# AaltoML/SLAM-module

Measured on AMD Instinct MI355X. Metric: frames/sec ORB extract+match (720p), higher is better.
Workload: dtype u8

## Files before the change

### slam-module_amd/csrc/describe_lanes.h

```cpp
#pragma once
#include <cstdint>

namespace describe_lanes {

constexpr int kWinRows = 45, kWinDwords = 12, kWinPieces = 9;
constexpr int kPatchRows = 32, kPatchDwords = 8, kHalfPatch = 15;
constexpr int kOriRow0 = 7, kOriDword0 = 2;

constexpr uint32_t win_pack(int lane) {
    uint32_t p = 0;
    for (int b = 0; b < 3; ++b) {
        const int i = lane + 64 * b;
        p |= (uint32_t)((i / kWinDwords) | ((4 * (i % kWinDwords)) << 4)) << (10 * b);
    }
    return p;
}
constexpr int win_row(uint32_t pack, int t) { return (int)((pack >> (10 * (t % 3))) & 15u) + 16 * (t / 3); }
constexpr int win_byte(uint32_t pack, int t) { return (int)((pack >> (10 * (t % 3) + 4)) & 63u); }
constexpr bool win_active(int lane, int t) { return t < kWinPieces - 1 || lane < kWinRows * kWinDwords - 64 * (kWinPieces - 1); }
constexpr int win_src_row(uint32_t pack, int lane, int t) { return win_active(lane, t) ? win_row(pack, t) : 16 * (t / 3); }
constexpr int win_src_byte(uint32_t pack, int lane, int t) { return win_active(lane, t) ? win_byte(pack, t) : 0; }
constexpr int win_slot(int lane, int t) { return lane + 64 * t; }
constexpr int kSlabDwords = kWinRows * kWinDwords + kPatchRows * kPatchDwords + 4;

constexpr int ori_base(int lane) { return ((lane >> 3) + kOriRow0) * kWinDwords + (lane & 7) + kOriDword0; }
constexpr int ori_src(int lane, int t) { return ori_base(lane) + 8 * kWinDwords * t; }
constexpr int ori_dst(int lane, int t) { return lane + 64 * t; }
constexpr bool ori_active(int lane, int t) { return t < 3 || lane < (kPatchRows - 1) * kPatchDwords - 64 * 3; }

inline uint32_t disc_mask(int lane, int t, const int *u_max) {
    const int i = ori_dst(lane, t), r = i >> 3, c4 = i & 7;
    if (r >= kPatchRows - 1) return 0u;
    uint32_t m = 0;
    for (int b = 0; b < 4; ++b) {
        const int u = 4 * c4 + b - kHalfPatch, v = r - kHalfPatch;
        if (u <= kHalfPatch && (u < 0 ? -u : u) <= u_max[v < 0 ? -v : v]) m |= 0xFFu << (8 * b);
    }
    return m;
}

constexpr uint32_t moment_col_weights(int lane) { return 0x03020100u + 0x04040404u * (uint32_t)(lane & 7); }
constexpr int moment_row_bias(int lane) { return (lane >> 3) - kHalfPatch + 24; }

#if defined(__HIP_DEVICE_COMPILE__)
__device__ __forceinline__ uint32_t sad_u8(uint32_t a, uint32_t acc) { return __builtin_amdgcn_sad_u8(a, 0u, acc); }
__device__ __forceinline__ uint32_t dot4_u8(uint32_t a, uint32_t w, uint32_t acc) { return __builtin_amdgcn_udot4(a, w, acc, false); }
#define DESCRIBE_LANES_FN __device__ __forceinline__
#else
inline uint32_t sad_u8(uint32_t a, uint32_t acc) { return acc + (a & 255u) + ((a >> 8) & 255u) + ((a >> 16) & 255u) + (a >> 24); }
inline uint32_t dot4_u8(uint32_t a, uint32_t w, uint32_t acc) {
    for (int b = 0; b < 4; ++b) acc += ((a >> (8 * b)) & 255u) * ((w >> (8 * b)) & 255u);
    return acc;
}
#define DESCRIBE_LANES_FN inline
#endif

DESCRIBE_LANES_FN void lane_moments(const uint32_t (&d)[4], uint32_t col_weights, int row_bias, int &m10, int &m01) {
    const uint32_t p0 = sad_u8(d[0], 0u), p1 = sad_u8(d[1], p0), p2 = sad_u8(d[2], p1), T = sad_u8(d[3], p2);
    const uint32_t D = dot4_u8(d[3], col_weights, dot4_u8(d[2], col_weights, dot4_u8(d[1], col_weights, dot4_u8(d[0], col_weights, 0u))));
    m10 = (int)D - kHalfPatch * (int)T;
    m01 = row_bias * (int)T - 8 * (int)(p0 + p1 + p2);
}
#undef DESCRIBE_LANES_FN

constexpr int kTapZeroSlot = 16;
constexpr int tap_slot(int lane, int t) {
    return ((unsigned)(lane - 16 * t) < 32u && (t < 2 || (lane & 15) <= 6)) ? lane - 16 * t : kTapZeroSlot;
}
inline void tap_table(uint32_t *out ) {
    const int w7[7] = {18, 34, 48, 56, 48, 34, 18};
    for (int i = 0; i < 64 * 4; ++i) out[i] = 0u;
    for (int tab = 0; tab < 2; ++tab)
        for (int dt = 0; dt < 2; ++dt)
            for (int n = 0; n < 16; ++n)
                for (int j = 0; j < 16; ++j) {
                    const int tap = 16 * dt + j - n - (tab == 0 ? 1 : 0);
                    const uint32_t v = (tap >= 0 && tap <= 6) ? (uint32_t)w7[tap] : 0u;
                    out[((tab * 2 + dt) * 16 + n) * 4 + j / 4] |= v << (8 * (j % 4));
                }
}

}
```

### slam-module_amd/csrc/hamming_fp4.h

```cpp
#pragma once
#include <stdint.h>

#if defined(__HIPCC__)
#define HM4_HD __host__ __device__ __forceinline__
#else
#define HM4_HD inline
#endif

constexpr uint32_t kHm4ScaleA = 0x80808080u;
constexpr uint32_t kHm4ScaleB = 0x83838383u;
constexpr int kHm4Steps = 4;

struct Hm4Slot { int step, half, dword, nibble; };
HM4_HD Hm4Slot hm4_slot(int bit) {
    const int wi = bit >> 5, b = bit & 31;
    return Hm4Slot{wi >> 1, wi & 1, b & 3, b >> 2};
}
HM4_HD uint32_t hm4_target_dword(uint32_t w, int j) { return (w >> j) & 0x11111111u; }
HM4_HD uint32_t hm4_query_dword(uint32_t w, int j) { return ((j < 3 ? w << (3 - j) : w) & 0x88888888u) | 0x22222222u; }
```

### slam-module_amd/csrc/match.hip

```cpp
#include "ms_internal.h"
#include "hamming_fp4.h"
#include <algorithm>
#include <cmath>
#include <cstring>
#include <vector>

namespace {

constexpr uint32_t kNone = 0xFFFFFFFFu;

__device__ __forceinline__ uint32_t hamming8(const uint32_t q[8], const uint4 a, const uint4 b) {
    uint32_t d = __popc(q[0] ^ a.x);
    d += __popc(q[1] ^ a.y); d += __popc(q[2] ^ a.z); d += __popc(q[3] ^ a.w);
    d += __popc(q[4] ^ b.x); d += __popc(q[5] ^ b.y); d += __popc(q[6] ^ b.z); d += __popc(q[7] ^ b.w);
    return d;
}

struct HamArgs {
    const uint32_t *q, *t;
    int32_t q_stride, t_stride;
    const int32_t *q_count, *t_count;
    const int32_t *pair_q, *pair_t;
    int32_t nq, nt;
    const int32_t *qb, *tb;
// ... 22 lines not shown
    int32_t my_bucket = 0;
    if (qi < nq) {
        const uint4 a = Q[2 * qi], b = Q[2 * qi + 1];
        qr[0] = a.x; qr[1] = a.y; qr[2] = a.z; qr[3] = a.w; qr[4] = b.x; qr[5] = b.y; qr[6] = b.z; qr[7] = b.w;
        if (MASKED && A.qb) my_bucket = A.qb[(uint64_t)qs * A.q_stride + qi];
    }
    uint32_t best = kNone, second = kNone;
    for (int base = 0; base < nt; base += 256) {
        __syncthreads();
        const int j = base + tid;
        if (j < nt) {
            s_t[tid][0] = T[2 * j]; s_t[tid][1] = T[2 * j + 1];
            if (MASKED) {
                s_b[tid] = A.tb ? A.tb[(uint64_t)ts * A.t_stride + j] : 0;
                s_v[tid] = A.tv ? A.tv[(uint64_t)ts * A.t_stride + j] : 1;
            }
        }
        __syncthreads();
        const int cnt = min(256, nt - base);
        for (int k = 0; k < cnt; ++k) {
            const uint32_t d = hamming8(qr, s_t[k][0], s_t[k][1]);
            uint32_t key = (d << 20) | (uint32_t)(base + k);
            if (MASKED) {
                const bool ok = s_v[k] != 0 && (!(A.qb && A.tb) || s_b[k] == my_bucket);
                key = ok ? key : kNone;
            }
            const uint32_t lo = min(best, key), hi = max(best, key);
            second = min(second, hi);
            best = lo;
        }
    }
    if (qi < A.q_stride) {
        const bool live = qi < nq;
        A.best_idx[o] = (!live || best == kNone) ? -1 : (int32_t)(best & 0xFFFFFu);
        A.best_dist[o] = (!live || best == kNone) ? (uint16_t)MS_HAMMING_MAX : (uint16_t)(best >> 20);
        A.second_dist[o] = (!live || second == kNone) ? (uint16_t)MS_HAMMING_MAX : (uint16_t)(second >> 20);
    }
}

typedef int v4i_t __attribute__((ext_vector_type(4)));
typedef int v8i_t __attribute__((ext_vector_type(8)));
typedef float v16f_t __attribute__((ext_vector_type(16)));
typedef unsigned short us2_t __attribute__((ext_vector_type(2)));
constexpr int kHmStage = 128;
static_assert(kHmStage == 128 || kHmStage == 256, "the expansion below gives every thread kHmStage / 128 sixteen-byte loads");

__device__ __forceinline__ void best2_push(uint32_t &best, uint32_t &second, uint32_t key) {
    const uint32_t lo = min(best, key), hi = max(best, key);
    second = min(second, hi);
    best = lo;
}
__device__ __forceinline__ v8i_t hm_operand(v4i_t v) { return v8i_t{v[0], v[1], v[2], v[3], 0, 0, 0, 0}; }

__global__ __launch_bounds__(256) void k_hamming_mfma(HamArgs A) {
    __shared__ __attribute__((aligned(16))) uint32_t s_a[kHmStage * 32];
    const int p = blockIdx.y, tid = threadIdx.x, lane = tid & 63, wave = __builtin_amdgcn_readfirstlane(tid >> 6);
    const int col = lane & 31, h = lane >> 5;
    const int qs = A.pair_q ? A.pair_q[p] : p, ts = A.pair_t ? A.pair_t[p] : p;
    const int nq = A.q_count ? min(A.q_count[qs], A.nq) : A.nq;
    const int nt = A.t_count ? min(A.t_count[ts], A.nt) : A.nt;
    if (blockIdx.x * 256 >= nq) {
        const int qi = blockIdx.x * 256 + tid;
        const uint64_t o = (uint64_t)p * A.q_stride + qi;
        if (qi < A.q_stride) { A.best_idx[o] = -1; A.best_dist[o] = MS_HAMMING_MAX; A.second_dist[o] = MS_HAMMING_MAX; }
        return;
    }
    const uint4 *Q = reinterpret_cast<const uint4 *>(A.q + (uint64_t)qs * A.q_stride * 8);
    const uint4 *T = reinterpret_cast<const uint4 *>(A.t + (uint64_t)ts * A.t_stride * 8);
    v4i_t bq[2][kHm4Steps];
    int popq[2];
    const uint32_t hmask = 0u - (uint32_t)h;
#pragma unroll
    for (int n = 0; n < 2; ++n) {
        const int qi = blockIdx.x * 256 + wave * 64 + n * 32 + col;
        uint4 lo = {0, 0, 0, 0}, hi = {0, 0, 0, 0};
        if (qi < nq) { lo = Q[2 * qi]; hi = Q[2 * qi + 1]; }
        const uint32_t w[8] = {lo.x, lo.y, lo.z, lo.w, hi.x, hi.y, hi.z, hi.w};
#pragma unroll
        for (int s = 0; s < kHm4Steps; ++s) {
            const uint32_t wq = (w[2 * s + 1] & hmask) | (w[2 * s] & ~hmask);
#pragma unroll
            for (int j = 0; j < 4; ++j) bq[n][s][j] = (int)hm4_query_dword(wq, j);
        }
        popq[n] = 0;
#pragma unroll
        for (int s = 0; s < 8; ++s) popq[n] += __popc(w[s]);
    }
    uint32_t best[2] = {kNone, kNone}, second[2] = {kNone, kNone};
    v16f_t tag;
#pragma unroll
    for (int r = 0; r < 16; ++r) tag[r] = 8388608.0f + 4096.0f + (float)r;
    for (int base = 0; base < nt; base += kHmStage) {
        __syncthreads();
#pragma unroll
        for (int it = 0; it < kHmStage / 128; ++it) {
            const int e = tid + 256 * it, tau = e % kHmStage, half = e / kHmStage, j = base + tau;
            uint4 v = {0, 0, 0, 0};
            if (j < nt) v = T[2 * j + half];
            const uint32_t w4[4] = {v.x, v.y, v.z, v.w};
#pragma unroll
            for (int k = 0; k < 4; ++k)
                *reinterpret_cast<v4i_t *>(&s_a[((tau >> 5) * kHm4Steps + 2 * half + (k >> 1)) * 256 + ((k & 1) * 32 + (tau & 31)) * 4]) =
                    v4i_t{(int)hm4_target_dword(w4[k], 0), (int)hm4_target_dword(w4[k], 1), (int)hm4_target_dword(w4[k], 2), (int)hm4_target_dword(w4[k], 3)};
        }
        __syncthreads();
        const int mtiles = min(kHmStage / 32, (nt - base + 31) >> 5);
        for (int m = 0; m < mtiles; ++m) {
            v16f_t acc[2];
            v4i_t a[kHm4Steps];
#pragma unroll
            for (int s = 0; s < kHm4Steps; ++s) a[s] = *reinterpret_cast<const v4i_t *>(&s_a[(m * kHm4Steps + s) * 256 + lane * 4]);
            __builtin_amdgcn_sched_barrier(0);
#pragma unroll
            for (int s = 0; s < kHm4Steps; ++s) {
                acc[0] = __builtin_amdgcn_mfma_scale_f32_32x32x64_f8f6f4(hm_operand(a[s]), hm_operand(bq[0][s]), s == 0 ? tag : acc[0], 4, 4, 0, (int)kHm4ScaleA, 0, (int)kHm4ScaleB);
                acc[1] = __builtin_amdgcn_mfma_scale_f32_32x32x64_f8f6f4(hm_operand(a[s]), hm_operand(bq[1][s]), s == 0 ? tag : acc[1], 4, 4, 0, (int)kHm4ScaleA, 0, (int)kHm4ScaleB);
            }
            const int row0 = base + m * 32 + 4 * h;
            if (base + m * 32 + 32 <= nt) {
                us2_t lb = {0xFFFF, 0xFFFF}, ls = {0xFFFF, 0xFFFF};
#pragma unroll
                for (int r = 0; r < 16; ++r) {
                    const uint32_t both = __builtin_amdgcn_perm(__float_as_uint(acc[1][r]), __float_as_uint(acc[0][r]), 0x05040100u);
                    const us2_t key = __builtin_bit_cast(us2_t, both);
                    const us2_t lo = __builtin_elementwise_min(lb, key), hi = __builtin_elementwise_max(lb, key);
                    ls = __builtin_elementwise_min(ls, hi);
                    lb = lo;
                }
#pragma unroll
                for (int n = 0; n < 2; ++n) {
                    const uint32_t kb = n ? lb.y : lb.x, ks = n ? ls.y : ls.x;
                    const uint32_t rb = kb & 15u, rs = ks & 15u;
                    best2_push(best[n], second[n], ((kb >> 4) << 20) + (uint32_t)row0 + (rb & 3u) + 8u * (rb >> 2));
                    second[n] = min(second[n], ((ks >> 4) << 20) + (uint32_t)row0 + (rs & 3u) + 8u * (rs >> 2));
                }
            } else {
#pragma unroll
                for (int n = 0; n < 2; ++n)
#pragma unroll
                    for (int r = 0; r < 16; ++r) {
                        const int row = row0 + (r & 3) + 8 * (r >> 2);
                        const uint32_t key = ((__float_as_uint(acc[n][r]) - (uint32_t)r) << 16) + (uint32_t)row;
                        best2_push(best[n], second[n], row < nt ? key : kNone);
                    }
            }
        }
    }
#pragma unroll
    for (int n = 0; n < 2; ++n) {
        const uint32_t ob = __shfl_xor(best[n], 32, 64), os = __shfl_xor(second[n], 32, 64);
        const uint32_t b = min(best[n], ob), s2 = min(max(best[n], ob), min(second[n], os));
        const int qi = blockIdx.x * 256 + wave * 64 + n * 32 + col;
        if (h == 0 && qi < A.q_stride) {
            const uint64_t o = (uint64_t)p * A.q_stride + qi;
            const bool live = qi < nq;
            A.best_idx[o] = (!live || b == kNone) ? -1 : (int32_t)(b & 0xFFFFFu);
            A.best_dist[o] = (!live || b == kNone) ? (uint16_t)MS_HAMMING_MAX : (uint16_t)((int)(b >> 20) - 256 + popq[n]);
            A.second_dist[o] = (!live || s2 == kNone) ? (uint16_t)MS_HAMMING_MAX : (uint16_t)((int)(s2 >> 20) - 256 + popq[n]);
        }
    }
}

__global__ __launch_bounds__(256) void k_ratio_test(const int32_t *__restrict__ bi, const uint16_t *__restrict__ bd, const uint16_t *__restrict__ sd,
                                                    int n, float ratio, int max_dist, int32_t *__restrict__ match) {
    const int i = blockIdx.x * 256 + threadIdx.x;
    if (i >= n) return;
    const unsigned b = bd[i], s = sd[i];
    bool ok = bi[i] >= 0 && b <= (unsigned)max_dist;
    if (ok && __fmul_rn(ratio, (float)s) < (float)b) ok = false;
    match[i] = ok ? bi[i] : -1;
}

__global__ __launch_bounds__(256) void k_descriptor_medoid(const uint32_t *__restrict__ pool, const int32_t *__restrict__ start,
                                                           const int32_t *__restrict__ idx, int cap,
                                                           int32_t *__restrict__ best_local, int32_t *__restrict__ best_pool) {
    extern __shared__ uint32_t s_dyn[];
    __shared__ uint32_t s_best;
    const int p = blockIdx.x, tid = threadIdx.x;
    const int s0 = start[p], n = start[p + 1] - s0;
    if (n <= 0 || n > cap) {
        const int code = n <= 0 ? -1 : -2;
        if (tid == 0) { if (best_local) best_local[p] = code; if (best_pool) best_pool[p] = code; }
        return;
    }
    uint32_t *s_desc = s_dyn;
    const int pitch = n | 1;
    uint16_t *s_mat = reinterpret_cast<uint16_t *>(s_dyn + 9 * n);
    for (int e = tid; e < 8 * n; e += 256) s_desc[9 * (e >> 3) + (e & 7)] = pool[8 * (size_t)idx[s0 + (e >> 3)] + (e & 7)];
    if (tid == 0) s_best = 0xffffffffu;
    __syncthreads();
    for (int e = tid; e < n * n; e += 256) {
        const int j = e / n, i = e - j * n;
        unsigned d = 0;
#pragma unroll
        for (int k = 0; k < 8; ++k) d += __popc(s_desc[9 * i + k] ^ s_desc[9 * j + k]);
        s_mat[i * pitch + j] = (uint16_t)d;
    }
    __syncthreads();
    const int kth = (n - 1) >> 1;
    for (int i = tid; i < n; i += 256) {
        int lo = 0, hi = 256;
        while (lo < hi) {
            const int mid = (lo + hi) >> 1;
            int cnt = 0;
            for (int j = 0; j < n; ++j) cnt += s_mat[i * pitch + j] <= mid;
            if (cnt > kth) hi = mid; else lo = mid + 1;
        }
        atomicMin(&s_best, ((uint32_t)lo << 16) | (uint32_t)i);
    }
    __syncthreads();
    if (tid == 0) {
// ... 607 lines not shown
            const int m = matched[i];
            if (m < 0) continue;
            const int bin = angle_bin(F1.angle[i], F2.angle[m]);
            atomicAdd(&s_hist[bin], 1);
            if (j < 8) {
#pragma unroll
                for (int jj = 0; jj < 8; ++jj) if (jj == j) bins[jj] = (int8_t)bin;
            }
        }
        __syncthreads();
        int v0 = -1, v1 = -1, v2 = -1;
        for (int rep = 0; rep < 3; ++rep) {
            int bb = -1, bc = -1;
            for (int k = 0; k < 30; ++k)
                if (k != v0 && k != v1 && s_hist[k] > bc) { bc = s_hist[k]; bb = k; }
            if (rep == 0) v0 = bb; else if (rep == 1) v1 = bb; else v2 = bb;
        }
        int removed = 0;
        for (int i = tid, j = 0; i < F1.n; i += 256, ++j) {
            int bin = -1;
            if (j < 8) {
#pragma unroll
                for (int jj = 0; jj < 8; ++jj) if (jj == j) bin = bins[jj];
                if (bin < 0) continue;
            } else {
                const int m = matched[i];
                if (m < 0) continue;
                bin = angle_bin(F1.angle[i], F2.angle[m]);
            }
            if (bin != v0 && bin != v1 && bin != v2) { matched[i] = -1; ++removed; }
        }
        if (removed) atomicAdd(&s_removed, removed);
        __syncthreads();
    }
    if (tid == 0) A.n_matches[p] = cnt[30] - s_removed;
}

}

extern "C" {

static int launch_hamming(ms_ctx *c, const HamArgs &A, int n_pairs) {
    MsRange range("match");
    if (A.nq < 0 || A.nt < 0 || n_pairs < 0 || A.nt >= (1 << 20) || n_pairs > 65535 || A.q_stride < A.nq || A.t_stride < A.nt)
        return ms_fail(c, MS_ERR_INVALID, "hamming search: size out of range");
    if (A.q_stride == 0 || n_pairs == 0) return MS_OK;
    if ((A.qb == nullptr) != (A.tb == nullptr)) return ms_fail(c, MS_ERR_INVALID, "hamming search: give both bucket arrays or neither");
    if (reinterpret_cast<uintptr_t>(A.q) % 16 || reinterpret_cast<uintptr_t>(A.t) % 16 || (A.q_stride * 32) % 16)
        return ms_fail(c, MS_ERR_INVALID, "hamming search: descriptors must be 16-byte aligned");
    MS_HIP(c, hipSetDevice(c->device));
    dim3 grid(ms_div_up(A.q_stride, 256), n_pairs);
    if (A.qb || A.tv) hipLaunchKernelGGL(k_hamming_best2<true>, grid, dim3(256), 0, c->stream, A);
    else if (c->hamming_path == 1) hipLaunchKernelGGL(k_hamming_best2<false>, grid, dim3(256), 0, c->stream, A);
    else hipLaunchKernelGGL(k_hamming_mfma, grid, dim3(256), 0, c->stream, A);
    MS_KERNEL_CHECK(c, "k_hamming_best2");
    return MS_OK;
}

int ms_hamming_set_path(ms_ctx *c, int path) {
    if (!c || path < 0 || path > 1) return MS_ERR_INVALID;
    c->hamming_path = path;
    return MS_OK;
}

int ms_hamming_best2(ms_ctx *c, const uint32_t *q, int nq, const uint32_t *t, int nt, int n_pairs,
                     const int32_t *q_bucket, const int32_t *t_bucket, const uint8_t *t_valid,
                     int32_t *best_idx, uint16_t *best_dist, uint16_t *second_dist) {
    if (!c || !q || !t || !best_idx || !best_dist || !second_dist) return MS_ERR_INVALID;
    HamArgs A{};
    A.q = q; A.t = t; A.q_stride = nq; A.t_stride = nt; A.nq = nq; A.nt = nt;
    A.qb = q_bucket; A.tb = t_bucket; A.tv = t_valid;
    A.best_idx = best_idx; A.best_dist = best_dist; A.second_dist = second_dist;
    return launch_hamming(c, A, n_pairs);
}

int ms_hamming_best2_sets(ms_ctx *c, const uint32_t *q_pool, int q_stride, const int32_t *q_count,
                          const uint32_t *t_pool, int t_stride, const int32_t *t_count,
                          const int32_t *pair_q, const int32_t *pair_t, int n_pairs,
                          int32_t *best_idx, uint16_t *best_dist, uint16_t *second_dist) {
    if (!c || !q_pool || !t_pool || !best_idx || !best_dist || !second_dist) return MS_ERR_INVALID;
    HamArgs A{};
    A.q = q_pool; A.t = t_pool; A.q_stride = q_stride; A.t_stride = t_stride; A.nq = q_stride; A.nt = t_stride;
    A.q_count = q_count; A.t_count = t_count; A.pair_q = pair_q; A.pair_t = pair_t;
    A.best_idx = best_idx; A.best_dist = best_dist; A.second_dist = second_dist;
    return launch_hamming(c, A, n_pairs);
}

int ms_hamming_candidates(ms_ctx *c, const uint32_t *q_desc, int nq, const uint32_t *t_desc, const int32_t *cand_start, const int32_t *cand_idx,
                          const uint8_t *t_skip, const int32_t *t_octave, int32_t *best_idx, uint16_t *best_dist, uint16_t *second_dist,
                          int32_t *best_octave, int32_t *second_octave, int32_t *second_idx) {
    if (!c || !q_desc || !t_desc || !cand_start || !cand_idx || !best_idx || !best_dist || !second_dist || nq < 0) return MS_ERR_INVALID;
    if (nq == 0) return MS_OK;
    if (reinterpret_cast<uintptr_t>(q_desc) % 16 || reinterpret_cast<uintptr_t>(t_desc) % 16) return ms_fail(c, MS_ERR_INVALID, "ms_hamming_candidates: descriptors must be 16-byte aligned");
    MS_HIP(c, hipSetDevice(c->device));
    hipLaunchKernelGGL(k_hamming_candidates<false>, dim3(ms_div_up(nq, 4)), dim3(256), 0, c->stream, q_desc, nq, t_desc, cand_start, cand_idx, t_skip, t_octave,
                       best_idx, best_dist, second_dist, best_octave, second_octave, second_idx);
    MS_KERNEL_CHECK(c, "k_hamming_candidates");
    return MS_OK;
}

int ms_hamming_candidates_topk(ms_ctx *c, const uint32_t *q_desc, int nq, const uint32_t *t_desc, const int32_t *cand_start, const int32_t *cand_idx,
                               const uint8_t *t_skip, const int32_t *t_octave, int32_t *top_idx, uint16_t *top_dist, int32_t *top_octave, int32_t *n_scored) {
    if (!c || !q_desc || !t_desc || !cand_start || !cand_idx || !top_idx || !top_dist || !top_octave || !n_scored || nq < 0) return MS_ERR_INVALID;
    if (nq == 0) return MS_OK;
    if (reinterpret_cast<uintptr_t>(q_desc) % 16 || reinterpret_cast<uintptr_t>(t_desc) % 16) return ms_fail(c, MS_ERR_INVALID, "ms_hamming_candidates_topk: descriptors must be 16-byte aligned");
    MsRange range("match");
    MS_HIP(c, hipSetDevice(c->device));
// ... 190 lines not shown
```

### slam-module_amd/csrc/orb.hip

```cpp
#include "ms_internal.h"
#include "fast_tiles.h"
#include "describe_lanes.h"
#include <cfloat>
#include <cmath>
#include <cstring>

namespace {

constexpr int kPatchRadius = MS_ORB_PATCH_RADIUS;
using describe_lanes::kHalfPatch;
constexpr int kMaxQuota = 4096;

struct LevelGeom {
    int32_t w, h, pitch, quota;
    int32_t min_dist;
    int32_t det_base;
    int32_t cand_cap;
    int32_t btiles_x, btile_base;
    uint32_t btiles_inv;
    uint64_t img_off, blur_off;
    uint64_t cand_off;
    float scale;
};

struct PyrGeom {
    int32_t levels, lk_level, fast_threshold, max_kpts, max_tracks, capacity;
    int32_t det_stride;
    int32_t width, height, btiles_total, ftiles_total;
    uint64_t slab_stride, cand_stride;
    int32_t umax[16];
    LevelGeom L[MS_MAX_LEVELS];
};

struct TileMap { int32_t base[MS_MAX_LEVELS + 1]; };
__device__ __forceinline__ int tile_level(const TileMap &tm, int levels, int t) {
    int l = 0;
#pragma unroll
    for (int k = 1; k < MS_MAX_LEVELS; ++k) l += t >= tm.base[k] ? 1 : 0;
    return l;
}

struct TileLevel { int32_t w, h, pitch, btiles_x, cand_cap; uint32_t btiles_inv; uint64_t img_off, blur_off, cand_off; float scale; int32_t det_base;
                   int32_t sel_k; };
struct TileLevels { TileLevel L[MS_MAX_LEVELS]; uint64_t slab_stride, cand_stride; int32_t levels, fast_threshold; };

struct FrameSrc {
    const uint8_t *lvl0;
    uint64_t lvl0_frame_stride;
    int32_t lvl0_pitch;
    uint8_t *slab;
};

__device__ __forceinline__ const uint8_t *level_ptr(const FrameSrc &s, const PyrGeom *g, int f, int l, int &pitch) {
    if (l == 0) { pitch = s.lvl0_pitch; return s.lvl0 + (uint64_t)f * s.lvl0_frame_stride; }
    pitch = g->L[l].pitch;
// ... 689 lines not shown
            }
        }
        const unsigned long long bo = __ballot(ok != 0);
        if (ln == 0 && wv < 4) s_w2[wv] = __popcll(bo);
        __syncthreads();
        int incl2 = __popcll(bo & ((2ull << ln) - 1ull)), out_chunk = 0;
        for (int w = 0; w < 4; ++w) { if (w < wv) incl2 += s_w2[w]; out_chunk += s_w2[w]; }
        if (ok) {
            const uint64_t slot = (uint64_t)f * g->det_stride + G.det_base + run + incl2 - 1;
            det_x[slot] = (int16_t)x; det_y[slot] = (int16_t)y; det_score[slot] = (uint8_t)sc;
        }
        __syncthreads();
        if (tid == 0) { s_run = run + out_chunk; s_kept = kept_before + kept_chunk; }
        __syncthreads();
    }
    if (tid == 0) { det_count[f * g->levels + l] = s_run; last_count[f * g->levels + l] = n_found; cand_count[f * g->levels + l] = 0; }
    if (score_hist && n_found > 0 && tid < 256) score_hist[((size_t)(f * g->levels + l) << 8) + tid] = 0;
}

__global__ __launch_bounds__(64) void k_tracks(const PyrGeom *g, const float *__restrict__ track_xy, const int32_t *__restrict__ track_id,
                                               const int32_t *__restrict__ n_tracks, const uint8_t *__restrict__ valid_mask,
                                               int16_t *__restrict__ trk_x, int16_t *__restrict__ trk_y, float *__restrict__ trk_px,
                                               float *__restrict__ trk_py, int32_t *__restrict__ trk_id, int32_t *__restrict__ trk_count) {
    const int f = blockIdx.x, lane = threadIdx.x;
    const int n = n_tracks ? min(n_tracks[f], g->max_tracks) : 0;
    const LevelGeom &G = g->L[g->lk_level];
    int run = 0;
    for (int base = 0; base < n; base += 64) {
        const int i = base + lane;
        bool ok = false; int x = 0, y = 0; float px = 0.f, py = 0.f;
        if (i < n) {
            px = track_xy[((uint64_t)f * g->max_tracks + i) * 2];
            py = track_xy[((uint64_t)f * g->max_tracks + i) * 2 + 1];
            x = __float2int_rn(__fdiv_rn(px, G.scale));
            y = __float2int_rn(__fdiv_rn(py, G.scale));
            ok = x >= kPatchRadius && y >= kPatchRadius && x < G.w - kPatchRadius && y < G.h - kPatchRadius;
            if (ok && valid_mask) {
                const int mx = __float2int_rn(px), my = __float2int_rn(py);
                ok = mx >= 0 && my >= 0 && mx < g->width && my < g->height && valid_mask[(uint64_t)my * g->width + mx] != 0;
            }
        }
        const unsigned long long bal = __ballot(ok);
        if (ok) {
            const uint64_t slot = (uint64_t)f * g->max_tracks + run + __popcll(bal & ((1ull << lane) - 1ull));
            trk_x[slot] = (int16_t)x; trk_y[slot] = (int16_t)y; trk_px[slot] = px; trk_py[slot] = py;
            trk_id[slot] = track_id ? track_id[(uint64_t)f * g->max_tracks + i] : i;
        }
        run += __popcll(bal);
    }
    if (lane == 0) trk_count[f] = run;
}


__device__ __forceinline__ float dev_fast_atan2(float y, float x) {
    const float p1 = 0.9997878412794807f * (float)(180 / 3.1415926535897932384626433832795);
    const float p3 = -0.3258083974640975f * (float)(180 / 3.1415926535897932384626433832795);
    const float p5 = 0.1555786518463281f * (float)(180 / 3.1415926535897932384626433832795);
    const float p7 = -0.04432655554792128f * (float)(180 / 3.1415926535897932384626433832795);
    const float ax = fabsf(x), ay = fabsf(y);
    float a, c, c2;
    if (ax >= ay) {
        c = __fdiv_rn(ay, __fadd_rn(ax, (float)DBL_EPSILON));
        c2 = __fmul_rn(c, c);
        a = __fmul_rn(__fadd_rn(__fmul_rn(__fadd_rn(__fmul_rn(__fadd_rn(__fmul_rn(p7, c2), p5), c2), p3), c2), p1), c);
    } else {
        c = __fdiv_rn(ax, __fadd_rn(ay, (float)DBL_EPSILON));
        c2 = __fmul_rn(c, c);
        a = __fsub_rn(90.f, __fmul_rn(__fadd_rn(__fmul_rn(__fadd_rn(__fmul_rn(__fadd_rn(__fmul_rn(p7, c2), p5), c2), p3), c2), p1), c));
    }
    if (x < 0) a = __fsub_rn(180.f, a);
    if (y < 0) a = __fsub_rn(360.f, a);
    return a;
}

__device__ __forceinline__ float dev_poly_cos(float v) {
    const float c1 = 0.99940307f, c2 = -0.49558072f, c3 = 0.03679168f;
    const float v2 = __fmul_rn(v, v);
    return __fadd_rn(c1, __fmul_rn(v2, __fadd_rn(c2, __fmul_rn(c3, v2))));
}
__device__ __forceinline__ float dev_cos(float v) {
    const float PI = 3.14159265358979f, PI_2 = PI / 2.0f, TWO_PI = 2.0f * PI, INV_TWO_PI = 1.0f / TWO_PI, THREE_PI_2 = 3.0f * PI_2;
    v = __fsub_rn(v, __fmul_rn((float)(int)floorf(__fmul_rn(v, INV_TWO_PI)), TWO_PI));
    v = (0.0f < v) ? v : -v;
    if (v < PI_2) return dev_poly_cos(v);
    else if (v < PI) return -dev_poly_cos(__fsub_rn(PI, v));
    else if (v < THREE_PI_2) return -dev_poly_cos(__fsub_rn(v, PI));
    else return dev_poly_cos(__fsub_rn(TWO_PI, v));
}
__device__ __forceinline__ float dev_sin(float v) { return dev_cos(__fsub_rn(3.14159265358979f / 2.0f, v)); }

__device__ __forceinline__ int wave_sum(int v) {
    return __builtin_amdgcn_readlane(wave_scan_add(v), 63);
}

__global__ __launch_bounds__(256) void k_slots(const int16_t *__restrict__ det_x, const int16_t *__restrict__ det_y, const int32_t *__restrict__ det_count,
                                               const int32_t *__restrict__ trk_count, uint2 *__restrict__ slot_tab, int32_t *__restrict__ out_count,
                                               TileLevels TL, int det_stride, int capacity) {
    const int l = blockIdx.x, f = blockIdx.y;
    int base = trk_count[f];
    for (int k = 0; k < l; ++k) base += det_count[f * TL.levels + k];
    const int cnt = det_count[f * TL.levels + l];
    const uint64_t s0 = (uint64_t)f * det_stride + TL.L[l].det_base;
    for (int i = threadIdx.x; i < cnt; i += 256)
        if (base + i < capacity) slot_tab[(uint64_t)f * capacity + base + i] = uint2{(uint32_t)(uint16_t)det_x[s0 + i] | ((uint32_t)(uint16_t)det_y[s0 + i] << 16), (uint32_t)l};
    if (l == TL.levels - 1 && threadIdx.x == 0) out_count[f] = min(base + cnt, capacity);
}

constexpr int kDescPerWave = 1;

struct DescKp { int x, y, oct, tid_out; float ox, oy; bool valid; };
typedef int v4i_t __attribute__((ext_vector_type(4)));
__device__ __forceinline__ void transpose4_rows(uint32_t (&r)[4]) {
    auto s = __builtin_amdgcn_permlane32_swap(r[0], r[2], false, false); r[0] = s[0]; r[2] = s[1];
    s = __builtin_amdgcn_permlane32_swap(r[1], r[3], false, false); r[1] = s[0]; r[3] = s[1];
    s = __builtin_amdgcn_permlane16_swap(r[0], r[1], false, false); r[0] = s[0]; r[1] = s[1];
    s = __builtin_amdgcn_permlane16_swap(r[2], r[3], false, false); r[2] = s[0]; r[3] = s[1];
}

__global__ __launch_bounds__(256) __attribute__((amdgpu_waves_per_eu(8, 8))) void k_describe(FrameSrc src, TileLevels TL, const uint4 *__restrict__ moment_tab, const float4 *__restrict__ pattern_f,
                                                  const uint2 *__restrict__ slot_tab, int capacity, int max_tracks, int lk_level,
                                                  const int16_t *__restrict__ trk_x, const int16_t *__restrict__ trk_y, const float *__restrict__ trk_px,
                                                  const float *__restrict__ trk_py, const int32_t *__restrict__ trk_id, const int32_t *__restrict__ trk_count,
                                                  float *__restrict__ out_x, float *__restrict__ out_y, float *__restrict__ out_angle,
                                                  int32_t *__restrict__ out_octave, uint32_t *__restrict__ out_desc, int32_t *__restrict__ out_track,
                                                  const int32_t *__restrict__ out_count) {
    const int f = blockIdx.y, lane = threadIdx.x & 63;
    const int slot0 = (blockIdx.x * 4 + __builtin_amdgcn_readfirstlane(threadIdx.x >> 6)) * kDescPerWave;
    __shared__ uint4 s_tab[64 + 256];
    if (threadIdx.x < 64) s_tab[threadIdx.x] = moment_tab[64 + threadIdx.x];
    s_tab[64 + threadIdx.x] = reinterpret_cast<const uint4 *>(pattern_f)[threadIdx.x];
    const uint4 dm = moment_tab[lane];
    const uint32_t dmask[4] = {dm.x, dm.y, dm.z, dm.w};
    const uint32_t wpack = reinterpret_cast<const uint32_t *>(moment_tab + 128)[lane];
    const int total = out_count[f], nt = trk_count[f];
    const uint2 ent = slot_tab[(uint64_t)f * capacity + min(slot0, capacity - 1)];
    __syncthreads();
    if (slot0 >= total) return;
    DescKp K[kDescPerWave];
#pragma unroll
    for (int k = 0; k < kDescPerWave; ++k) {
        const int slot = slot0 + k;
        K[k].valid = slot < total;
// ... 46 lines not shown
        {
            const uint32_t *ob = win + describe_lanes::ori_base(lane);
            uint32_t d[4];
#pragma unroll
            for (int t = 0; t < 4; ++t) d[t] = (describe_lanes::ori_active(lane, t) ? ob[8 * describe_lanes::kWinDwords * t] : 0u) & dmask[t];
            int p10, p01;
            describe_lanes::lane_moments(d, describe_lanes::moment_col_weights(lane), describe_lanes::moment_row_bias(lane), p10, p01);
            m10[k] = wave_sum(p10); m01[k] = wave_sum(p01);
        }
        {
            const int n = lane & 15, q = lane >> 4;
            auto taps = [&](int base, int t) { return __builtin_bit_cast(v4i_t, s_tab[base + describe_lanes::tap_slot(lane, t)]); };
            v4i_t Aw[3], Vb[3];
#pragma unroll
            for (int m = 0; m < 3; ++m) {
                uint4 a4 = *reinterpret_cast<const uint4 *>(win + (16 * m + n) * 12 + 4 * q);
                a4.x ^= 0x80808080u; a4.y ^= 0x80808080u; a4.z ^= 0x80808080u; a4.w ^= 0x80808080u;
                Aw[m] = __builtin_bit_cast(v4i_t, a4);
                Vb[m] = taps(32, m);
            }
#pragma unroll
            for (int t = 0; t < 3; ++t) {
                const v4i_t Hb = taps(0, t), zero = {0, 0, 0, 0};
                uint32_t hd[4], ld[4];
#pragma unroll
                for (int m = 0; m < 3; ++m) {
                    const v4i_t T = __builtin_amdgcn_mfma_i32_16x16x64_i8(Aw[m], Hb, zero, 0, 0, 0);
                    const uint32_t x01 = __builtin_amdgcn_perm((uint32_t)T[1], (uint32_t)T[0], 0x04000501u);
                    const uint32_t x23 = __builtin_amdgcn_perm((uint32_t)T[3], (uint32_t)T[2], 0x04000501u);
                    hd[m] = __builtin_amdgcn_perm(x23, x01, 0x05040100u);
                    ld[m] = __builtin_amdgcn_perm(x23, x01, 0x07060302u) ^ 0x80808080u;
                }
                hd[3] = 0; ld[3] = 0;
                transpose4_rows(hd); transpose4_rows(ld);
                const v4i_t A2h = {(int)hd[0], (int)hd[1], (int)hd[2], (int)hd[3]}, A2l = {(int)ld[0], (int)ld[1], (int)ld[2], (int)ld[3]};
#pragma unroll
                for (int yt = 0; yt < 3; ++yt) {
                    v4i_t acc = {33024, 33024, 33024, 33024};
                    acc = __builtin_amdgcn_mfma_i32_16x16x64_i8(A2h, Vb[yt], acc, 0, 0, 0);
                    acc <<= 8;
                    acc = __builtin_amdgcn_mfma_i32_16x16x64_i8(A2l, Vb[yt], acc, 0, 0, 0);
                    const int y = 16 * yt + n;
                    if (y < 39 && 4 * t + q < 10)
                        pb[y * 10 + 4 * t + q] = __builtin_amdgcn_perm((uint32_t)acc[1], (uint32_t)acc[0], 0x0C0C0602u) | __builtin_amdgcn_perm((uint32_t)acc[3], (uint32_t)acc[2], 0x06020C0Cu);
                }
            }
        }
    }
    __builtin_amdgcn_fence(__ATOMIC_ACQ_REL, "wavefront");
    __builtin_amdgcn_wave_barrier();
    float angle_deg[kDescPerWave], ca[kDescPerWave], sa[kDescPerWave];
#pragma unroll
    for (int k = 0; k < kDescPerWave; ++k) {
        angle_deg[k] = dev_fast_atan2((float)m01[k], (float)m10[k]);
        const float angle = (float)__dmul_rn((double)angle_deg[k], M_PI / 180.0);
        ca[k] = dev_cos(angle); sa[k] = dev_sin(angle);
    }
    unsigned long long bits[kDescPerWave][4];
#pragma unroll
    for (int q = 0; q < 4; ++q) {
        const float4 pt = __builtin_bit_cast(float4, s_tab[64 + q * 64 + lane]);
        const float x1 = pt.x, y1 = pt.y, x2 = pt.z, y2 = pt.w;
#pragma unroll
        for (int k = 0; k < kDescPerWave; ++k) {
            const uint8_t *pb = reinterpret_cast<const uint8_t *>(&s_patch[wv][k][0]);
            const int r1 = __float2int_rn(__fadd_rn(__fmul_rn(x1, sa[k]), __fmul_rn(y1, ca[k])));
            const int c1 = __float2int_rn(__fsub_rn(__fmul_rn(x1, ca[k]), __fmul_rn(y1, sa[k])));
            const int r2 = __float2int_rn(__fadd_rn(__fmul_rn(x2, sa[k]), __fmul_rn(y2, ca[k])));
            const int c2 = __float2int_rn(__fsub_rn(__fmul_rn(x2, ca[k]), __fmul_rn(y2, sa[k])));
            bits[k][q] = __ballot(pb[(r1 + kPatchRadius) * 40 + (c1 + kPatchRadius)] < pb[(r2 + kPatchRadius) * 40 + (c2 + kPatchRadius)]);
        }
    }
#pragma unroll
    for (int k = 0; k < kDescPerWave; ++k) {
        if (!K[k].valid) continue;
        const uint64_t o = (uint64_t)f * capacity + slot0 + k;
        if (lane < 8) out_desc[o * 8 + lane] = (uint32_t)(bits[k][lane >> 1] >> ((lane & 1) * 32));
        if (lane == 0) { out_x[o] = K[k].ox; out_y[o] = K[k].oy; out_angle[o] = angle_deg[k]; out_octave[o] = K[k].oct; out_track[o] = K[k].tid_out; }
    }
}

}

struct ms_orb {
    ms_ctx *ctx = nullptr;
    ms_orb_config cfg{};
    PyrGeom geom{};
    PyrGeom *d_geom = nullptr;
    TileMap blur_tiles{};
    uint2 *d_ftile_tab = nullptr;
    TileLevels tile_levels{};
    uint8_t *d_slab = nullptr;
    uint32_t *d_cand = nullptr;
    int32_t *d_cand_count = nullptr, *d_det_count = nullptr, *d_trk_count = nullptr;
    size_t cand_count_bytes = 0, score_hist_bytes = 0;
    uint32_t *d_score_hist = nullptr;
    int32_t *d_last_count = nullptr;
    int16_t *d_det_x = nullptr, *d_det_y = nullptr, *d_trk_x = nullptr, *d_trk_y = nullptr;
    uint8_t *d_det_score = nullptr, *d_mask = nullptr;
    float *d_trk_px = nullptr, *d_trk_py = nullptr, *d_track_xy = nullptr;
    int32_t *d_trk_id = nullptr, *d_track_id = nullptr, *d_n_tracks = nullptr;
    float *d_x = nullptr, *d_y = nullptr, *d_angle = nullptr;
    int32_t *d_octave = nullptr, *d_track = nullptr, *d_count = nullptr;
    uint2 *d_slot_tab = nullptr;
    uint32_t *d_desc = nullptr;
    int16_t *d_xtab[MS_MAX_LEVELS] = {nullptr}, *d_ytab[MS_MAX_LEVELS] = {nullptr};
    bool wide[MS_MAX_LEVELS] = {false};
    uint4 *d_moment_tab = nullptr;
    float4 *d_pattern_f = nullptr;
    bool profiling = false;
    bool blur_valid = false;
    static constexpr int kProfRing = 128;
    hipEvent_t evr[kProfRing][MS_ORB_STAGES + 1] = {{nullptr}};
    hipEvent_t *ev = evr[0];
    long long prof_calls = 0;
    hipStream_t copy_stream = nullptr;
    hipEvent_t ev_copied[4] = {nullptr}, ev_free[4] = {nullptr}, ev_end = nullptr;
    int chunked_frames = 0;
    bool end_recorded = false;
    FrameSrc last_src{};
    int last_frames = 0;
    bool lvl0_in_slab = false;
    uint64_t lvl0_off = 0;
// ... 528 lines not shown
```

Baseline: 165,200.

## Pack hamming best-2 keys into float accumulator and branchless steer trig

Adds a KEY32 variant of the MFMA Hamming kernel. A larger B scale and a per-row start tag make each float accumulator bit pattern a sortable key holding both distance and row, so best/second tracking reduces to min/max on raw bits with a per-tile age adjustment. This replaces the previous 16-bit packed-tag path when the target count fits. Separately, descriptor steering becomes branchless: lanes 0 and 1 each compute one of cos and sin, which are then broadcast with readlane, and mul24 is used for the moment and patch index arithmetic. These changes add key-decoding complexity and some reliance on exact float encoding.

```diff
diff --git a/slam-module_amd/csrc/describe_lanes.h b/slam-module_amd/csrc/describe_lanes.h
--- a/slam-module_amd/csrc/describe_lanes.h
+++ b/slam-module_amd/csrc/describe_lanes.h
@@ -45,8 +45,10 @@
 #if defined(__HIP_DEVICE_COMPILE__)
 __device__ __forceinline__ uint32_t sad_u8(uint32_t a, uint32_t acc) { return __builtin_amdgcn_sad_u8(a, 0u, acc); }
 __device__ __forceinline__ uint32_t dot4_u8(uint32_t a, uint32_t w, uint32_t acc) { return __builtin_amdgcn_udot4(a, w, acc, false); }
+__device__ __forceinline__ int mul_small(int a, int b) { return __mul24(a, b); }
 #define DESCRIBE_LANES_FN __device__ __forceinline__
 #else
+inline int mul_small(int a, int b) { return a * b; }
 inline uint32_t sad_u8(uint32_t a, uint32_t acc) { return acc + (a & 255u) + ((a >> 8) & 255u) + ((a >> 16) & 255u) + (a >> 24); }
 inline uint32_t dot4_u8(uint32_t a, uint32_t w, uint32_t acc) {
     for (int b = 0; b < 4; ++b) acc += ((a >> (8 * b)) & 255u) * ((w >> (8 * b)) & 255u);
@@ -59,7 +61,7 @@
     const uint32_t p0 = sad_u8(d[0], 0u), p1 = sad_u8(d[1], p0), p2 = sad_u8(d[2], p1), T = sad_u8(d[3], p2);
     const uint32_t D = dot4_u8(d[3], col_weights, dot4_u8(d[2], col_weights, dot4_u8(d[1], col_weights, dot4_u8(d[0], col_weights, 0u))));
     m10 = (int)D - kHalfPatch * (int)T;
-    m01 = row_bias * (int)T - 8 * (int)(p0 + p1 + p2);
+    m01 = mul_small(row_bias, (int)T) - 8 * (int)(p0 + p1 + p2);
 }
 #undef DESCRIBE_LANES_FN
 
diff --git a/slam-module_amd/csrc/describe_steer.h b/slam-module_amd/csrc/describe_steer.h
--- /dev/null
+++ b/slam-module_amd/csrc/describe_steer.h
@@ -0,0 +1,63 @@
+#pragma once
+#include <cfloat>
+#include <cmath>
+#include <cstdint>
+
+#if defined(__HIPCC__)
+#define DSTEER_HD __host__ __device__ __forceinline__
+#else
+#define DSTEER_HD inline
+#endif
+#if defined(__HIP_DEVICE_COMPILE__)
+#define DSTEER_ADD(a, b) __fadd_rn(a, b)
+#define DSTEER_SUB(a, b) __fsub_rn(a, b)
+#define DSTEER_MUL(a, b) __fmul_rn(a, b)
+#define DSTEER_DIV(a, b) __fdiv_rn(a, b)
+#else
+#define DSTEER_ADD(a, b) ((a) + (b))
+#define DSTEER_SUB(a, b) ((a) - (b))
+#define DSTEER_MUL(a, b) ((a) * (b))
+#define DSTEER_DIV(a, b) ((a) / (b))
+#endif
+
+namespace describe_steer {
+
+DSTEER_HD float fast_atan2(float y, float x) {
+    const float p1 = 0.9997878412794807f * (float)(180 / 3.1415926535897932384626433832795);
+    const float p3 = -0.3258083974640975f * (float)(180 / 3.1415926535897932384626433832795);
+    const float p5 = 0.1555786518463281f * (float)(180 / 3.1415926535897932384626433832795);
+    const float p7 = -0.04432655554792128f * (float)(180 / 3.1415926535897932384626433832795);
+    const float ax = fabsf(x), ay = fabsf(y);
+    const bool swap = !(ax >= ay);
+    const float lo = swap ? ax : ay, hi = swap ? ay : ax;
+    const float c = DSTEER_DIV(lo, DSTEER_ADD(hi, (float)DBL_EPSILON));
+    const float c2 = DSTEER_MUL(c, c);
+    float a = DSTEER_MUL(DSTEER_ADD(DSTEER_MUL(DSTEER_ADD(DSTEER_MUL(DSTEER_ADD(DSTEER_MUL(p7, c2), p5), c2), p3), c2), p1), c);
+    if (swap) a = DSTEER_SUB(90.f, a);
+    if (x < 0) a = DSTEER_SUB(180.f, a);
+    if (y < 0) a = DSTEER_SUB(360.f, a);
+    return a;
+}
+
+DSTEER_HD float deg_to_rad(float deg) { return (float)((double)deg * (M_PI / 180.0)); }
+
+DSTEER_HD float poly_cos(float v) {
+    const float c1 = 0.99940307f, c2 = -0.49558072f, c3 = 0.03679168f;
+    const float v2 = DSTEER_MUL(v, v);
+    return DSTEER_ADD(c1, DSTEER_MUL(v2, DSTEER_ADD(c2, DSTEER_MUL(c3, v2))));
+}
+DSTEER_HD float cos_approx(float v) {
+    const float PI = 3.14159265358979f, PI_2 = PI / 2.0f, TWO_PI = 2.0f * PI, INV_TWO_PI = 1.0f / TWO_PI, THREE_PI_2 = 3.0f * PI_2;
+    v = DSTEER_SUB(v, DSTEER_MUL((float)(int)floorf(DSTEER_MUL(v, INV_TWO_PI)), TWO_PI));
+    v = (0.0f < v) ? v : -v;
+    const bool q0 = v < PI_2, q1 = v < PI, q2 = v < THREE_PI_2;
+    const float lhs = q0 ? v : q1 ? PI : q2 ? v : TWO_PI;
+    const float rhs = q1 ? v : q2 ? PI : v;
+    const float arg = q0 ? v : DSTEER_SUB(lhs, rhs);
+    const float r = poly_cos(arg);
+    return (!q0 && q2) ? -r : r;
+}
+DSTEER_HD float sin_argument(float v) { return DSTEER_SUB(3.14159265358979f / 2.0f, v); }
+DSTEER_HD float sin_approx(float v) { return cos_approx(sin_argument(v)); }
+
+}
diff --git a/slam-module_amd/csrc/hamming_fp4.h b/slam-module_amd/csrc/hamming_fp4.h
--- a/slam-module_amd/csrc/hamming_fp4.h
+++ b/slam-module_amd/csrc/hamming_fp4.h
@@ -18,3 +18,24 @@
 }
 HM4_HD uint32_t hm4_target_dword(uint32_t w, int j) { return (w >> j) & 0x11111111u; }
 HM4_HD uint32_t hm4_query_dword(uint32_t w, int j) { return ((j < 3 ? w << (3 - j) : w) & 0x88888888u) | 0x22222222u; }
+
+constexpr uint32_t kHm4ScaleBKey = 0x8C8C8C8Cu;
+constexpr int kHmKeyShift = 13;
+constexpr uint32_t kHmKeyS = 1u << kHmKeyShift;
+constexpr int kHmKeyMaxRows = (int)kHmKeyS;
+constexpr uint32_t kHmKeyBase = 0x4B000000u;
+constexpr uint32_t kHmKeyNone = 0xFFFFFFFFu;
+
+HM4_HD int hm_key_row_in_tile(int r, int h) { return (r & 3) + 8 * (r >> 2) + 4 * h; }
+HM4_HD float hm_key_start(int r, int h) { return 8388608.0f + (float)(256u * kHmKeyS) + (float)((int)kHmKeyS - 32 + hm_key_row_in_tile(r, h)); }
+HM4_HD uint32_t hm_key_umin(uint32_t a, uint32_t b) { return a < b ? a : b; }
+HM4_HD uint32_t hm_key_umax(uint32_t a, uint32_t b) { return a < b ? b : a; }
+HM4_HD void hm_key_age(uint32_t &best, uint32_t &second) { best -= 32u; second -= 32u; }
+HM4_HD void hm_key_push2(uint32_t &best, uint32_t &second, uint32_t k0, uint32_t k1) {
+    const uint32_t med = hm_key_umin(hm_key_umax(k0, k1), hm_key_umax(hm_key_umin(k0, k1), best));
+    second = hm_key_umin(second, med);
+    best = hm_key_umin(hm_key_umin(best, k0), k1);
+}
+HM4_HD bool hm_key_empty(uint32_t key) { return key >= 0x80000000u; }
+HM4_HD int hm_key_dot256(uint32_t key) { return (int)((key - kHmKeyBase) >> kHmKeyShift); }
+HM4_HD int hm_key_row(uint32_t key, int tiles_seen) { return (int)((key - kHmKeyBase) & (kHmKeyS - 1u)) - (int)kHmKeyS + 32 * tiles_seen; }
diff --git a/slam-module_amd/csrc/match.hip b/slam-module_amd/csrc/match.hip
--- a/slam-module_amd/csrc/match.hip
+++ b/slam-module_amd/csrc/match.hip
@@ -98,8 +98,10 @@
 }
 __device__ __forceinline__ v8i_t hm_operand(v4i_t v) { return v8i_t{v[0], v[1], v[2], v[3], 0, 0, 0, 0}; }
 
+template <bool KEY32>
 __global__ __launch_bounds__(256) void k_hamming_mfma(HamArgs A) {
     __shared__ __attribute__((aligned(16))) uint32_t s_a[kHmStage * 32];
+    constexpr int kScaleB = (int)(KEY32 ? kHm4ScaleBKey : kHm4ScaleB);
     const int p = blockIdx.y, tid = threadIdx.x, lane = tid & 63, wave = __builtin_amdgcn_readfirstlane(tid >> 6);
     const int col = lane & 31, h = lane >> 5;
     const int qs = A.pair_q ? A.pair_q[p] : p, ts = A.pair_t ? A.pair_t[p] : p;
@@ -135,7 +137,7 @@
     uint32_t best[2] = {kNone, kNone}, second[2] = {kNone, kNone};
     v16f_t tag;
 #pragma unroll
-    for (int r = 0; r < 16; ++r) tag[r] = 8388608.0f + 4096.0f + (float)r;
+    for (int r = 0; r < 16; ++r) tag[r] = KEY32 ? hm_key_start(r, h) : 8388608.0f + 4096.0f + (float)r;
     for (int base = 0; base < nt; base += kHmStage) {
         __syncthreads();
 #pragma unroll
@@ -159,11 +161,26 @@
             __builtin_amdgcn_sched_barrier(0);
 #pragma unroll
             for (int s = 0; s < kHm4Steps; ++s) {
-                acc[0] = __builtin_amdgcn_mfma_scale_f32_32x32x64_f8f6f4(hm_operand(a[s]), hm_operand(bq[0][s]), s == 0 ? tag : acc[0], 4, 4, 0, (int)kHm4ScaleA, 0, (int)kHm4ScaleB);
-                acc[1] = __builtin_amdgcn_mfma_scale_f32_32x32x64_f8f6f4(hm_operand(a[s]), hm_operand(bq[1][s]), s == 0 ? tag : acc[1], 4, 4, 0, (int)kHm4ScaleA, 0, (int)kHm4ScaleB);
+                acc[0] = __builtin_amdgcn_mfma_scale_f32_32x32x64_f8f6f4(hm_operand(a[s]), hm_operand(bq[0][s]), s == 0 ? tag : acc[0], 4, 4, 0, (int)kHm4ScaleA, 0, kScaleB);
+                acc[1] = __builtin_amdgcn_mfma_scale_f32_32x32x64_f8f6f4(hm_operand(a[s]), hm_operand(bq[1][s]), s == 0 ? tag : acc[1], 4, 4, 0, (int)kHm4ScaleA, 0, kScaleB);
             }
             const int row0 = base + m * 32 + 4 * h;
-            if (base + m * 32 + 32 <= nt) {
+            if constexpr (KEY32) {
+                hm_key_age(best[0], second[0]); hm_key_age(best[1], second[1]);
+                if (base + m * 32 + 32 <= nt) {
+#pragma unroll
+                    for (int n = 0; n < 2; ++n)
+#pragma unroll
+                        for (int r = 0; r < 16; r += 2) hm_key_push2(best[n], second[n], __float_as_uint(acc[n][r]), __float_as_uint(acc[n][r + 1]));
+                } else {
+#pragma unroll
+                    for (int n = 0; n < 2; ++n)
+#pragma unroll
+                        for (int r = 0; r < 16; r += 2)
+                            hm_key_push2(best[n], second[n], row0 + hm_key_row_in_tile(r, 0) < nt ? __float_as_uint(acc[n][r]) : kNone,
+                                         row0 + hm_key_row_in_tile(r + 1, 0) < nt ? __float_as_uint(acc[n][r + 1]) : kNone);
+                }
+            } else if (base + m * 32 + 32 <= nt) {
                 us2_t lb = {0xFFFF, 0xFFFF}, ls = {0xFFFF, 0xFFFF};
 #pragma unroll
                 for (int r = 0; r < 16; ++r) {
@@ -200,9 +217,16 @@
         if (h == 0 && qi < A.q_stride) {
             const uint64_t o = (uint64_t)p * A.q_stride + qi;
             const bool live = qi < nq;
-            A.best_idx[o] = (!live || b == kNone) ? -1 : (int32_t)(b & 0xFFFFFu);
-            A.best_dist[o] = (!live || b == kNone) ? (uint16_t)MS_HAMMING_MAX : (uint16_t)((int)(b >> 20) - 256 + popq[n]);
-            A.second_dist[o] = (!live || s2 == kNone) ? (uint16_t)MS_HAMMING_MAX : (uint16_t)((int)(s2 >> 20) - 256 + popq[n]);
+            if constexpr (KEY32) {
+                const bool nb = !live || hm_key_empty(b), ns = !live || hm_key_empty(s2);
+                A.best_idx[o] = nb ? -1 : (int32_t)hm_key_row(b, (nt + 31) >> 5);
+                A.best_dist[o] = nb ? (uint16_t)MS_HAMMING_MAX : (uint16_t)(hm_key_dot256(b) - 256 + popq[n]);
+                A.second_dist[o] = ns ? (uint16_t)MS_HAMMING_MAX : (uint16_t)(hm_key_dot256(s2) - 256 + popq[n]);
+            } else {
+                A.best_idx[o] = (!live || b == kNone) ? -1 : (int32_t)(b & 0xFFFFFu);
+                A.best_dist[o] = (!live || b == kNone) ? (uint16_t)MS_HAMMING_MAX : (uint16_t)((int)(b >> 20) - 256 + popq[n]);
+                A.second_dist[o] = (!live || s2 == kNone) ? (uint16_t)MS_HAMMING_MAX : (uint16_t)((int)(s2 >> 20) - 256 + popq[n]);
+            }
         }
     }
 }
@@ -916,7 +940,8 @@
     dim3 grid(ms_div_up(A.q_stride, 256), n_pairs);
     if (A.qb || A.tv) hipLaunchKernelGGL(k_hamming_best2<true>, grid, dim3(256), 0, c->stream, A);
     else if (c->hamming_path == 1) hipLaunchKernelGGL(k_hamming_best2<false>, grid, dim3(256), 0, c->stream, A);
-    else hipLaunchKernelGGL(k_hamming_mfma, grid, dim3(256), 0, c->stream, A);
+    else if (A.nt <= kHmKeyMaxRows) hipLaunchKernelGGL(k_hamming_mfma<true>, grid, dim3(256), 0, c->stream, A);
+    else hipLaunchKernelGGL(k_hamming_mfma<false>, grid, dim3(256), 0, c->stream, A);
     MS_KERNEL_CHECK(c, "k_hamming_best2");
     return MS_OK;
 }
diff --git a/slam-module_amd/csrc/orb.hip b/slam-module_amd/csrc/orb.hip
--- a/slam-module_amd/csrc/orb.hip
+++ b/slam-module_amd/csrc/orb.hip
@@ -1,6 +1,7 @@
 #include "ms_internal.h"
 #include "fast_tiles.h"
 #include "describe_lanes.h"
+#include "describe_steer.h"
 #include <cfloat>
 #include <cmath>
 #include <cstring>
@@ -796,42 +797,6 @@
 }
 
 
-__device__ __forceinline__ float dev_fast_atan2(float y, float x) {
-    const float p1 = 0.9997878412794807f * (float)(180 / 3.1415926535897932384626433832795);
-    const float p3 = -0.3258083974640975f * (float)(180 / 3.1415926535897932384626433832795);
-    const float p5 = 0.1555786518463281f * (float)(180 / 3.1415926535897932384626433832795);
-    const float p7 = -0.04432655554792128f * (float)(180 / 3.1415926535897932384626433832795);
-    const float ax = fabsf(x), ay = fabsf(y);
-    float a, c, c2;
-    if (ax >= ay) {
-        c = __fdiv_rn(ay, __fadd_rn(ax, (float)DBL_EPSILON));
-        c2 = __fmul_rn(c, c);
-        a = __fmul_rn(__fadd_rn(__fmul_rn(__fadd_rn(__fmul_rn(__fadd_rn(__fmul_rn(p7, c2), p5), c2), p3), c2), p1), c);
-    } else {
-        c = __fdiv_rn(ax, __fadd_rn(ay, (float)DBL_EPSILON));
-        c2 = __fmul_rn(c, c);
-        a = __fsub_rn(90.f, __fmul_rn(__fadd_rn(__fmul_rn(__fadd_rn(__fmul_rn(__fadd_rn(__fmul_rn(p7, c2), p5), c2), p3), c2), p1), c));
-    }
-    if (x < 0) a = __fsub_rn(180.f, a);
-    if (y < 0) a = __fsub_rn(360.f, a);
-    return a;
-}
-
-__device__ __forceinline__ float dev_poly_cos(float v) {
-    const float c1 = 0.99940307f, c2 = -0.49558072f, c3 = 0.03679168f;
-    const float v2 = __fmul_rn(v, v);
-    return __fadd_rn(c1, __fmul_rn(v2, __fadd_rn(c2, __fmul_rn(c3, v2))));
-}
-__device__ __forceinline__ float dev_cos(float v) {
-    const float PI = 3.14159265358979f, PI_2 = PI / 2.0f, TWO_PI = 2.0f * PI, INV_TWO_PI = 1.0f / TWO_PI, THREE_PI_2 = 3.0f * PI_2;
-    v = __fsub_rn(v, __fmul_rn((float)(int)floorf(__fmul_rn(v, INV_TWO_PI)), TWO_PI));
-    v = (0.0f < v) ? v : -v;
-    if (v < PI_2) return dev_poly_cos(v);
-    else if (v < PI) return -dev_poly_cos(__fsub_rn(PI, v));
-    else if (v < THREE_PI_2) return -dev_poly_cos(__fsub_rn(v, PI));
-    else return dev_poly_cos(__fsub_rn(TWO_PI, v));
-}
-__device__ __forceinline__ float dev_sin(float v) { return dev_cos(__fsub_rn(3.14159265358979f / 2.0f, v)); }
 
 __device__ __forceinline__ int wave_sum(int v) {
     return __builtin_amdgcn_readlane(wave_scan_add(v), 63);
@@ -984,9 +949,11 @@
     float angle_deg[kDescPerWave], ca[kDescPerWave], sa[kDescPerWave];
 #pragma unroll
     for (int k = 0; k < kDescPerWave; ++k) {
-        angle_deg[k] = dev_fast_atan2((float)m01[k], (float)m10[k]);
-        const float angle = (float)__dmul_rn((double)angle_deg[k], M_PI / 180.0);
-        ca[k] = dev_cos(angle); sa[k] = dev_sin(angle);
+        angle_deg[k] = describe_steer::fast_atan2((float)m01[k], (float)m10[k]);
+        const float angle = describe_steer::deg_to_rad(angle_deg[k]);
+        const float cs = describe_steer::cos_approx(lane == 1 ? describe_steer::sin_argument(angle) : angle);
+        ca[k] = __builtin_bit_cast(float, __builtin_amdgcn_readlane(__builtin_bit_cast(int, cs), 0));
+        sa[k] = __builtin_bit_cast(float, __builtin_amdgcn_readlane(__builtin_bit_cast(int, cs), 1));
     }
     unsigned long long bits[kDescPerWave][4];
 #pragma unroll
@@ -1000,7 +967,8 @@
             const int c1 = __float2int_rn(__fsub_rn(__fmul_rn(x1, ca[k]), __fmul_rn(y1, sa[k])));
             const int r2 = __float2int_rn(__fadd_rn(__fmul_rn(x2, sa[k]), __fmul_rn(y2, ca[k])));
             const int c2 = __float2int_rn(__fsub_rn(__fmul_rn(x2, ca[k]), __fmul_rn(y2, sa[k])));
-            bits[k][q] = __ballot(pb[(r1 + kPatchRadius) * 40 + (c1 + kPatchRadius)] < pb[(r2 + kPatchRadius) * 40 + (c2 + kPatchRadius)]);
+            const uint32_t i1 = __umul24((uint32_t)(r1 + kPatchRadius), 40u) + (uint32_t)(c1 + kPatchRadius), i2 = __umul24((uint32_t)(r2 + kPatchRadius), 40u) + (uint32_t)(c2 + kPatchRadius);
+            bits[k][q] = __ballot(pb[i1] < pb[i2]);
         }
     }
 #pragma unroll
```

Result: faster. 169,400 (median of 6 runs) (+2.5%).
